# Efrat19/flink

Hardware: AMD Instinct MI355X
Metric: events/sec keyed sliding-window agg at 1/2/4/8 GPUs; % of HBM roofline (higher is better)
Workload: dtype int64

## Files before the change

flink_amd/csrc/gw_kernels.h:

```cpp
#pragma once
#include "gw_device.h"

namespace gw {

struct PaneTable {
    int64_t* base;
    int64_t cap;
    int64_t nreg;
    int64_t region_words;
    int32_t log2S;
    int32_t rb1;
    int32_t nsub;
    int32_t ring;
    int32_t words;
    int32_t agg;
    int32_t has_mask;
    int32_t mask_shift;
};

GW_HD int64_t pt_S(const PaneTable& t) { return (int64_t)1 << t.log2S; }
GW_HD int64_t* pt_region(const PaneTable& t, int64_t r) { return t.base + r * t.region_words; }
GW_HD int64_t* pt_key(const PaneTable& t, int64_t g) {
    return pt_region(t, g >> t.log2S) + (g & (pt_S(t) - 1));
}
// ... 113 lines not shown
    int32_t sr_bits;
    uint64_t apply_mask;
    uint64_t c_mask;
    const int64_t* c_rbeg;
    const uint32_t* c_r_row;
    const int64_t* c_r_base;
    int64_t* c_key;
    int32_t cur_empty;
    int64_t tile0;
    int64_t ntiles;
    int64_t ngroups;
    int32_t p2_group;
    int64_t* p1_key;
    int64_t* p1_a0;
    int64_t* p1_a1;
    uint8_t* p1_pos;
    uint32_t* p1_row;
    uint32_t* p2_desc;
    int64_t* p2_off;
    int64_t* p2_roff;
    int64_t* rbeg;
    int64_t* bk_off;
    int64_t* e_key;
    int64_t* e_a0;
    int64_t* e_a1;
    uint8_t* e_pos;
    uint32_t* r_row;
    int64_t* r_base;
    unsigned long long* batch_occ;
    DevStatus* st_host;
    unsigned long long st_seq;
    uint64_t ring_fresh;
    int32_t stale;
};

#ifndef GW_PART_TILE
#define GW_PART_TILE 4096
#endif
constexpr int kPartTile = GW_PART_TILE;
constexpr int kPartBuckets = 256;
constexpr int kRgnMaxRegions = 65536;
constexpr int kMaxGroup = 256;

struct MergeArgs {
    const int64_t* i_key;
    const int64_t* i_pane;
    const int64_t* i_a0;
    const int64_t* i_a1;
    int64_t n;
    int64_t b;
    int32_t b_pos;
    PaneTable t;
    int64_t* d_key;
    int64_t* d_pane;
    int64_t* d_a0;
    int64_t* d_a1;
    DevStatus* st;
};

constexpr uint32_t kOvTimer = 1;
constexpr uint32_t kOvDead = 2;
struct Overlay {
    const int32_t* head;
    const int64_t* key;
    const int64_t* k;
    const int64_t* a0;
// ... 63 lines not shown
    const int64_t* d_pane;
    const int64_t* d_a0;
    const int64_t* d_a1;
    int64_t n_def;
    int32_t max_p, kg_lo, kg_hi;
    int64_t* o_key;
    int64_t* o_pane;
    int64_t* o_a0;
    int64_t* o_a1;
    int32_t* o_kg;
    unsigned long long* n_out;
};
hipError_t launch_snap_collect(const SnapArgs& a, hipStream_t s);

hipError_t launch_table_init(const PaneTable& t, hipStream_t s);
hipError_t launch_overlay_attach(const PaneTable& t, const Overlay& ov, int32_t* head, DevStatus* st, hipStream_t s);
hipError_t launch_ingest(const IngestArgs& a, int path, int unroll, hipStream_t s);
hipError_t launch_region_p1(const IngestArgs& a, hipStream_t s, hipEvent_t e0 = nullptr, hipEvent_t e1 = nullptr);
hipError_t launch_publish_status(const IngestArgs& a, hipStream_t s);
hipError_t launch_region_flush(const IngestArgs& a, hipStream_t s, hipEvent_t e0 = nullptr, hipEvent_t e1 = nullptr);
hipError_t launch_region_collect(const IngestArgs& a, hipStream_t s);
int region_group(int d1_bits);
hipError_t launch_merge_deferred(const MergeArgs& a, hipStream_t s);
hipError_t launch_refire(const RefireArgs& a, hipStream_t s);
hipError_t launch_refire_keys(int mode, const int64_t* src, int64_t base, uint64_t* k, uint32_t* v, int64_t n,
                              hipStream_t s);
hipError_t launch_deferred_min(const int64_t* pane, int64_t n, DevStatus* st, hipStream_t s);
hipError_t launch_fire(const FireArgs& a, hipStream_t s, hipEvent_t e0 = nullptr, hipEvent_t e1 = nullptr);
struct FireGuard {
    unsigned long long expect_ndef;
    int64_t o_cap;
    int64_t nwin;
    int64_t reset_rows;
};
hipError_t launch_fire_guard(DevStatus* st, const FireGuard& g, hipStream_t s);
hipError_t launch_clean_stale(const PaneTable& t, uint64_t pmask, hipStream_t s);
hipError_t launch_evict(const EvictArgs& a, hipStream_t s);
hipError_t launch_rehash(const PaneTable& o, const PaneTable& n, DevStatus* st, hipStream_t s);
hipError_t launch_status_set(DevStatus* st, int word, unsigned long long v, int shard_field, hipStream_t s);
hipError_t launch_count_live(const PaneTable& t, unsigned long long* out, hipStream_t s);

hipError_t launch_key_groups(int64_t n, const int64_t* key, const int32_t* key_hash, int32_t max_p,
                             int32_t p, int32_t* kg, int32_t* owner, hipStream_t s);
int64_t partition_scratch_bytes(int64_t n, int32_t p);
hipError_t launch_check_keys(int64_t n, const int64_t* key, const int32_t* key_hash, int32_t max_p, int32_t kg_lo,
                             int32_t kg_hi, int check_range, unsigned long long* out, hipStream_t s);
constexpr int32_t kPartRegionMaxOwners = 16;
hipError_t launch_partition_regions(int64_t n, const int64_t* key, const int32_t* key_hash, const int64_t* ts,
                                    const int64_t* val, int32_t max_p, int32_t p, int64_t cap, int64_t* key_out,
                                    int64_t* ts_out, int64_t* val_out, int32_t* hash_out, const PackGeom* pack,
                                    uint64_t* packed_out, int64_t* counts, void* scratch, hipStream_t s,
                                    int turn = -1, int32_t nd_max = 0, int unstable = 0);
int64_t partition_regions_scratch_bytes(int64_t cap, int32_t nd);
hipError_t launch_partition(int64_t n, const int64_t* key, const int32_t* key_hash, const int64_t* ts,
                            const int64_t* val, int32_t max_p, int32_t p, int64_t* key_out,
                            int64_t* ts_out, int64_t* val_out, int64_t* counts, void* scratch,
                            hipStream_t s, int32_t* hash_out = nullptr, const PackGeom* pack = nullptr,
                            uint64_t* packed_out = nullptr);
hipError_t launch_select_lookup(int64_t n, const int64_t* sel, int64_t want, const int64_t* idx, const int64_t* dict,
                                int64_t dict_n, const int64_t* ts, int64_t* key_out, int64_t* ts_out, void* scratch,
                                hipStream_t s);
size_t select_lookup_scratch_bytes(int64_t n);
hipError_t launch_unpack(int64_t n, const uint64_t* w, const PackGeom& g, int64_t* key, int64_t* ts, int64_t* val,
                         hipStream_t s);

struct KeyHashMap {
    int64_t* key = nullptr;
    int32_t* hash = nullptr;
// ... 11 lines not shown
```

flink_amd/csrc/gw_pane.hip:

```cpp
#include <hip/hip_ext.h>
#include <type_traits>
#include "gw_kernels.h"

#include <algorithm>
#include <mutex>
#include <vector>

namespace gw {

template <int AGG>
__device__ __forceinline__ constexpr bool uses_mask() {
    return !(AGG == GW_COUNT || AGG == GW_AVG_I64 || AGG == GW_AVG_F64);
}

template <int AGG>
__device__ __forceinline__ uint64_t presence(const PaneTable& t, int64_t g) {
    if constexpr (uses_mask<AGG>()) {
        return pt_mask_get(t, g);
    } else {
        uint64_t m = 0;
        for (int r = 0; r < t.ring; ++r)
            if (pt_cell(t, g, r)[t.words - 1] != 0) m |= 1ull << r;
        return m;
    }
// ... 1304 lines not shown
        spills = marked;
    }
    __syncthreads();
    {
        const long2* sk = reinterpret_cast<const long2*>(lkeys);
        long2* dk = reinterpret_cast<long2*>(gkeys);
        for (int64_t w = threadIdx.x; w < S / 2; w += blockDim.x) {
            const int64_t line = w >> 3;
            if (s_kdirty[line >> 5] & (1u << (line & 31))) {
                const long2 v = sk[w];
                dk[w] = long2{slot_unhash((uint64_t)v.x), slot_unhash((uint64_t)v.y)};
            }
        }
    }
    if constexpr (M) copy_words((long long*)gmask, (const long long*)lmask, MW);
    for (int ai = 0; ai < 2; ++ai) {
        const int p = ai ? act1 : act0;
        if (p < 0) continue;
        copy_words((long long*)pt_cell(a.t, r << a.t.log2S, p), lcell + (int64_t)ai * S * W, S * W);
    }
    spills = wave_sum(spills);
    if (__lane_id() == 0 && spills) atomicAdd(&a.st->spills, spills);
    block_commit(a.st, 0, ins, flags, 0);
}

constexpr uint32_t kK32Empty = 0xffffffffu;
constexpr uint32_t kK32Foreign = 0xfffffffeu;
constexpr int kNarMaxF = 4;
constexpr int kNarMaxSlots = kNarMaxF * 2048;
constexpr int kNarLoadU = 4;
#ifndef GW_NAR_DEPTH
#define GW_NAR_DEPTH 2
#endif

__device__ __forceinline__ uint32_t k32_of(int64_t k) {
    return k == kEmptyKey ? kK32Empty : ((uint64_t)k < (uint64_t)kK32Foreign ? (uint32_t)k : kK32Foreign);
}

template <int AGG, bool STALE>
__global__ void __launch_bounds__(kApplyThreads) GW_APPLY_ATTR k_rgn_apply_nar(IngestArgs a) {
    if constexpr (!cmp_agg<AGG>()) {
        return;
    } else {
    extern __shared__ __attribute__((aligned(16))) unsigned char smem[];
    constexpr bool M = uses_mask<AGG>();
    constexpr bool N4 = AGG == GW_COUNT;
    constexpr int W = AGG == GW_AVG_I64 ? 2 : 1;
    __shared__ uint32_t r_cnt[kApplyRuns], r_src[kApplyRuns];
    __shared__ uint32_t s_kdirty[kNarMaxSlots / 16 / 32];
    __shared__ uint32_t s_pos;
    const int F = 1 << a.sr_bits;
    const int S = (int)pt_S(a.t), FS = F * S;
    const int l2S = a.t.log2S;
    const int64_t ncol = a.t.nsub >> a.sr_bits;
    const int64_t sr = blockIdx.x;
    const int64_t bucket = sr / ncol, col = sr - bucket * ncol;
    const int64_t rb0 = a.cur_empty ? 0 : a.rbeg[bucket], re0 = a.cur_empty ? 0 : a.rbeg[bucket + 1];
    const int64_t rb1 = a.c_mask ? a.c_rbeg[bucket] : 0, re1 = a.c_mask ? a.c_rbeg[bucket + 1] : 0;
    const int lane = threadIdx.x & 63, wave = threadIdx.x >> 6, nw = blockDim.x >> 6;
    uint32_t* lkeys = reinterpret_cast<uint32_t*>(smem);
    uint8_t* lmask = reinterpret_cast<uint8_t*>(lkeys + FS);
    long long* lcell = reinterpret_cast<long long*>(lmask + (M ? FS : 0));
    uint32_t* qk = reinterpret_cast<uint32_t*>(lcell + (int64_t)FS * W) + wave * kApplyQ;
    int32_t* qv = reinterpret_cast<int32_t*>(lcell + (int64_t)FS * W) + nw * kApplyQ + wave * kApplyQ;
    int qn = 0;
    const unsigned long long cur_pos = a.cur_empty ? 0ull : (*(volatile unsigned long long*)a.batch_occ) & a.apply_mask;
    struct List {
        const uint32_t* rows;
        const int64_t* rbase;
        const uint64_t* rk;
        const uint32_t* rk32;
        int64_t rb, re;
        unsigned long long pos;
    };
    const List list0{a.r_row, a.r_base, reinterpret_cast<const uint64_t*>(a.e_key),
                     reinterpret_cast<const uint32_t*>(a.e_key), rb0, re0, cur_pos & 0xffull};
    const List list1{a.c_r_row, a.c_r_base, reinterpret_cast<const uint64_t*>(a.c_key),
                     reinterpret_cast<const uint32_t*>(a.c_key), rb1, re1, a.c_mask & 0xffull};

    if (threadIdx.x == 0) s_pos = 0;
    for (int i = threadIdx.x; i < kNarMaxSlots / 16 / 32; i += blockDim.x) s_kdirty[i] = 0;
    __syncthreads();
    {
        uint32_t any = 0;
        for (int l = 0; l < 2; ++l) {
            const List L = l ? list1 : list0;
            for (int64_t rnd = L.rb + threadIdx.x; rnd < L.re; rnd += blockDim.x)
                for (unsigned long long pm = L.pos; pm; pm &= pm - 1) {
                    const int p = __ffsll((long long)pm) - 1;
                    if (L.rows[rnd * kPartBuckets + ((col << 3) | p)] & 0xffffu) any |= 1u << p;
                }
        }
        any = (uint32_t)wave_ior(any);
        if (lane == 0 && any) atomicOr(&s_pos, any);
    }
    __syncthreads();
    const uint32_t pmask = s_pos;
    if (!pmask) return;

    {
        const int nk2 = FS / 2, nm16 = M ? FS / 16 : 0, tot = nk2 + nm16;
        for (int w0 = threadIdx.x; w0 < tot; w0 += kNarLoadU * blockDim.x) {
            long2 v[kNarLoadU];
#pragma unroll
            for (int u = 0; u < kNarLoadU; ++u) {
                const int w = w0 + u * blockDim.x;
                v[u] = long2{0, 0};
                if (w < nk2) {
                    const int d = w >> (l2S - 1), j = w & (S / 2 - 1);
                    v[u] = reinterpret_cast<const long2*>(pt_region(a.t, sr * F + d))[j];
                } else if (w < tot) {
                    const int wm_ = w - nk2, d = wm_ >> (l2S - 4), j = wm_ & (S / 16 - 1);
                    v[u] = reinterpret_cast<const long2*>(pt_mask_base(a.t, sr * F + d))[j];
                }
            }
#pragma unroll
            for (int u = 0; u < kNarLoadU; ++u) {
                const int w = w0 + u * blockDim.x;
                if (w < nk2) {
                    reinterpret_cast<uint2*>(lkeys)[w] = uint2{k32_of(v[u].x), k32_of(v[u].y)};
                } else if (w < tot) {
                    reinterpret_cast<long2*>(lmask)[w - nk2] = v[u];
                }
            }
        }
    }
    unsigned long long ins = 0, flags = 0, spills = 0;

    auto probe_insert = [&](uint32_t k, uint64_t h) -> int {
        const int d = F > 1 ? (int)(pt_sub(a.t, h) & (F - 1)) : 0;
        uint32_t* kd = lkeys + d * S;
// ... 226 lines not shown
        for (int l = 0; l < 2; ++l) {
            const List L = l ? list1 : list0;
            for (unsigned long long pm = L.pos & pmask; pm; pm &= pm - 1) {
                const int p = __ffsll((long long)pm) - 1;
                const int64_t ccol = (col << 3) | p;
                for (int64_t rnd = L.rb + wave; rnd < L.re; rnd += nw) {
                    const uint32_t d = L.rows[rnd * kPartBuckets + ccol];
                    const int64_t src = L.rbase[rnd] + (d >> 16);
                    for (uint32_t k = lane; k < (d & 0xffffu); k += 64) {
                        const uint64_t r = N4 ? (uint64_t)L.rk32[src + k] : L.rk[src + k];
                        const uint32_t kk = N4 ? (uint32_t)(r >> 4) : (uint32_t)r;
                        const uint64_t h = slot_hash((int64_t)kk);
                        const int dd = F > 1 ? (int)(pt_sub(a.t, h) & (F - 1)) : 0;
                        int j = (int)(h & (uint64_t)(S - 1) & ~(uint64_t)(kProbeGroup - 1));
                        bool present = false;
                        for (int q = 0; q < S; ++q) {
                            const uint32_t x = lkeys[dd * S + j];
                            if (x == kk) { present = true; break; }
                            if (x == kK32Empty) break;
                            j = (j + 1) & (S - 1);
                        }
                        if (!present) {
                            if constexpr (N4) const_cast<uint32_t*>(L.rk32)[src + k] = (uint32_t)r | kNarSpill;
                            else const_cast<uint64_t*>(L.rk)[src + k] = r | ((uint64_t)kNarSpill << 32);
                            marked++;
                        }
                    }
                }
            }
        }
        spills = marked;
    }
    __syncthreads();
    if constexpr (M) {
        const int per = S / 16, lper = l2S - 4;
        for (int w = threadIdx.x; w < FS / 16; w += blockDim.x) {
            const int d = w >> lper;
            reinterpret_cast<long2*>(pt_mask_base(a.t, sr * F + d))[w - d * per] = reinterpret_cast<const long2*>(lmask)[w];
        }
    }
    for (int j = threadIdx.x; j < FS; j += blockDim.x) {
        const int line = j >> 4;
        if ((s_kdirty[line >> 5] >> (line & 31)) & 1u) {
            const uint32_t k = lkeys[j];
            if (k != kK32Foreign) {
                const int d = j >> l2S;
                pt_region(a.t, sr * F + d)[j - d * S] = k == kK32Empty ? kEmptyKey : (int64_t)k;
            }
        }
    }
    spills = wave_sum(spills);
    if (__lane_id() == 0 && spills) atomicAdd(&a.st->spills, spills);
    block_commit(a.st, 0, ins, flags, 0);
    }
}

template <int AGG>
__global__ void __launch_bounds__(256) k_rgn_collect_nar2(IngestArgs a) {
    constexpr bool N4 = AGG == GW_COUNT;
    const bool carry = blockIdx.y == 1;
    if (carry ? !a.c_mask : a.cur_empty) return;
    const int nb1 = 1 << a.d1_bits;
    const int64_t n = carry ? a.c_rbeg[kPartBuckets + 1 + nb1] : a.bk_off[nb1];
    int64_t* rk = carry ? a.c_key : a.e_key;
    uint32_t* rk32 = reinterpret_cast<uint32_t*>(rk);
    const int64_t stride = (int64_t)gridDim.x * blockDim.x;
    for (int64_t base = blockIdx.x * (int64_t)blockDim.x; base < n; base += stride) {
        const int64_t i = base + threadIdx.x;
        bool spill = false;
        int64_t key = 0, pane = 0, c0 = 0;
        if (i < n) {
            const uint64_t w = N4 ? (uint64_t)rk32[i] : (uint64_t)rk[i];
            const uint32_t lo = N4 ? (uint32_t)w : (uint32_t)(w >> 32);
            if (nar_spilled(lo)) {
                spill = true;
                if (N4) rk32[i] = (uint32_t)w & ~kNarSpill;
                else rk[i] = (int64_t)(w & ~((uint64_t)kNarSpill << 32));
                key = N4 ? nar_key32((uint32_t)w) : nar_key(w);
                c0 = N4 ? 1 : nar_val(w);
                const int64_t rel = ((int64_t)nar_pos(lo) - a.b_pos + a.t.ring) % a.t.ring;
                pane = a.p_late + (int64_t)a.delta + rel;
            }
        }
        defer_write(a, spill, key, pane, c0, 1);
    }
}
// ... 472 lines not shown
        load(A, c0);
        for (int64_t base = c0; base < c1; base += 2 * step) {
            const bool more = base + step < c1;
            if (more) load(B, base + step);
            fold(A, base);
            if (!more) break;
            if (base + 2 * step < c1) load(A, base + 2 * step);
            fold(B, base + step);
        }
    }
    flush();
}

template <int AGG>
__global__ void __launch_bounds__(256) k_clean_stale(PaneTable t, uint64_t pm) {
    if constexpr (uses_mask<AGG>()) {
        const int64_t id0 = identity0(AGG);
        for (int64_t g = blockIdx.x * (int64_t)blockDim.x + threadIdx.x; g < t.cap; g += (int64_t)gridDim.x * blockDim.x) {
            const uint64_t m = pt_mask_get(t, g);
            for (uint64_t q = pm & ~m; q; q &= q - 1) pt_cell(t, g, __ffsll((long long)q) - 1)[0] = id0;
        }
    }
}

__global__ void __launch_bounds__(64) k_fire_guard(DevStatus* st, FireGuard g) {
    const int lane = threadIdx.x;
    unsigned long long flags = 0, used = 0;
    for (int i = lane; i < kShards; i += 64) {
        flags |= st->sh[i].flags;
        used += st->sh[i].ins;
    }
    flags = wave_ior(flags);
    used = wave_sum(used);
    if (lane == 0) {
        if (g.reset_rows) st->rows = 0;
        const unsigned long long rows = g.reset_rows ? 0ull : st->rows;
        const bool skip = st->spills != 0 || st->wide_vals != 0 ||
                          (flags & (GW_DF_TABLE_FULL | GW_DF_NO_TS | GW_DF_RANGE)) != 0 ||
                          st->n_deferred != g.expect_ndef ||
                          (int64_t)rows + g.nwin * ((int64_t)used + 1) > g.o_cap;
        st->fire_skip = skip ? 1ull : 0ull;
        st->fire_rows0 = rows;
    }
}

template <int AGG>
__global__ void __launch_bounds__(256) k_evict(EvictArgs a) {
    const int64_t nslots = a.t.cap + 1;
    const int64_t stride = (int64_t)gridDim.x * blockDim.x;
    const int64_t id0 = identity0(AGG);
    const int W = a.t.words;
    if (blockIdx.x == 0 && threadIdx.x < kShards) atomicAnd(&a.st->sh[threadIdx.x].occ, ~a.emask);
    for (int64_t base = blockIdx.x * (int64_t)blockDim.x; base < nslots; base += stride) {
        const int64_t g = base + threadIdx.x;
        uint64_t m = 0;
        int64_t key = 0;
        if (g < nslots) {
            key = *pt_key(a.t, g);
            m = presence<AGG>(a.t, g) & a.emask;
        }
        unsigned long long off = wave_reserve_n(&a.st->n_deferred, (unsigned)__popcll(m));
        if (m) {
            if constexpr (uses_mask<AGG>()) pt_mask_put(a.t, g, pt_mask_get(a.t, g) & ~a.emask);
            while (m) {
                const int pos = __ffsll((long long)m) - 1;
                m &= m - 1;
                int64_t* c = pt_cell(a.t, g, pos);
                a.d_key[off] = key;
                a.d_pane[off] = a.pane_of_pos[pos];
                a.d_a0[off] = c[0];
                a.d_a1[off] = W == 2 ? c[1] : 0;
                off++;
                c[0] = id0;
                if (W == 2) c[1] = 0;
            }
// ... 231 lines not shown
        GW_TLAUNCH(k_rgn_plan1, dim3((unsigned)a.ngroups), dim3(256), 0, s, e0, nullptr, a);                   \
        hipLaunchKernelGGL(k_rgn_plan2, dim3((unsigned)nb1), dim3(256), 0, s, a);                              \
        hipLaunchKernelGGL(k_rgn_plan3, dim3(1), dim3(256), 0, s, a);                                          \
        hipLaunchKernelGGL((k_rgn_p2<A, CM>), dim3((unsigned)(a.ngroups * nb1)), dim3(kPartThreads), part_lds, s, \
                           a);                                                                                  \
    }                                                                                                           \
    GW_TLAUNCH((k_rgn_apply<A, CM>), dim3((unsigned)a.t.nreg), dim3(kApplyThreads), apply_lds, s,               \
               single ? e0 : nullptr, e1, a)
#define L(A)                        \
    if (a.fmt == kFmtNar) {         \
        L2(A, kFmtNar);             \
    } else if (a.fmt == kFmtCmp) {  \
        L2(A, kFmtCmp);             \
    } else {                        \
        L2(A, kFmtWide);            \
    }
    if (a.fmt == kFmtNar && a.nar2) {
        const int F = 1 << a.sr_bits;
        const int64_t FS = (int64_t)F * S;
        const bool M = a.t.has_mask != 0;
        const size_t lds = (size_t)FS * 4 + (M ? (size_t)FS : 0) + (size_t)FS * a.t.words * 8 +
                           (size_t)(kApplyThreads / 64) * kApplyQ * 8;
#define LN(A)                                                                                                   \
    lds_opt_in((const void*)k_rgn_p2<A, kFmtNar>, part_lds);                                                   \
    lds_opt_in((const void*)k_rgn_apply_nar<A, true>, lds);                                                   \
    lds_opt_in((const void*)k_rgn_apply_nar<A, false>, lds);                                                  \
    if (!a.cur_empty) {                                                                                         \
        GW_TLAUNCH(k_rgn_plan1, dim3((unsigned)a.ngroups), dim3(256), 0, s, e0, nullptr, a);                   \
        hipLaunchKernelGGL(k_rgn_plan2, dim3((unsigned)nb1), dim3(256), 0, s, a);                              \
        hipLaunchKernelGGL(k_rgn_plan3, dim3(1), dim3(256), 0, s, a);                                          \
        hipLaunchKernelGGL((k_rgn_p2<A, kFmtNar>), dim3((unsigned)(a.ngroups * nb1)), dim3(kPartThreads), part_lds, \
                           s, a);                                                                               \
    }                                                                                                           \
    if (a.stale)                                                                                                \
        GW_TLAUNCH((k_rgn_apply_nar<A, true>), dim3((unsigned)(a.t.nreg >> a.sr_bits)), dim3(kApplyThreads), lds, \
                   s, a.cur_empty ? e0 : nullptr, e1, a);                                                       \
    else                                                                                                        \
        GW_TLAUNCH((k_rgn_apply_nar<A, false>), dim3((unsigned)(a.t.nreg >> a.sr_bits)), dim3(kApplyThreads),     \
                   lds, s, a.cur_empty ? e0 : nullptr, e1, a)
        GW_AGG_SWITCH(a.t.agg, LN);
#undef LN
        return hipGetLastError();
    }
    GW_AGG_SWITCH(a.t.agg, L);
#undef L
#undef L2
    return hipGetLastError();
}

hipError_t launch_region_collect(const IngestArgs& a, hipStream_t s) {
    const int64_t n = a.ntiles * kPartTile;
#define L(A)                                                                                         \
    if (a.fmt == kFmtNar && a.nar2)                                                                  \
        hipLaunchKernelGGL(k_rgn_collect_nar2<A>, dim3(grid_for(n), 2), dim3(256), 0, s, a);        \
    else if (a.fmt == kFmtNar)                                                                       \
        hipLaunchKernelGGL(k_rgn_collect_nar<A>, dim3((unsigned)a.t.nreg), dim3(256), 0, s, a);     \
    else if (a.fmt == kFmtCmp)                                                                       \
        hipLaunchKernelGGL(k_rgn_collect_cmp<A>, dim3((unsigned)a.t.nreg), dim3(256), 0, s, a);     \
    else                                                                                             \
        hipLaunchKernelGGL(k_rgn_collect<A>, dim3(grid_for(n)), dim3(256), 0, s, a)
    GW_AGG_SWITCH(a.t.agg, L);
#undef L
    return hipGetLastError();
}

hipError_t launch_merge_deferred(const MergeArgs& a, hipStream_t s) {
#define L(A) hipLaunchKernelGGL(k_merge_deferred<A>, dim3(grid_for(a.n)), dim3(256), 0, s, a)
// ... 31 lines not shown
    if (a.ov.head == nullptr && npos >= 1 && npos <= 6 && a.nwin <= 255 &&
        (int64_t)a.nwin * kF2Threads * 2 <= kF2Stage) {
        const bool av = a.t.agg == GW_AVG_I64 || a.t.agg == GW_AVG_F64;
        const int64_t tile = (int64_t)kF2Threads * (av ? 1 : 2);
        const int fg = (int)std::min<int64_t>(1024, std::max<int64_t>(1, (a.t.cap + 1 + tile - 1) / tile));
#define F2(A, NPV) \
    GW_TLAUNCH((k_fire2<A, NPV, (A == GW_AVG_I64 || A == GW_AVG_F64) ? 1 : 2>), dim3(fg), dim3(kF2Threads), 0, s, e0, e1, a)
#define L(A)                      \
    switch (npos) {               \
    case 1: F2(A, 1); break;      \
    case 2: F2(A, 2); break;      \
    case 3: F2(A, 3); break;      \
    case 4: F2(A, 4); break;      \
    case 5: F2(A, 5); break;      \
    default: F2(A, 6); break;     \
    }
        GW_AGG_SWITCH(a.t.agg, L);
#undef L
#undef F2
        return hipGetLastError();
    }
    const int fg = (int)std::min<int64_t>(1024, std::max<int64_t>(1, (a.t.cap + 1 + 255) / 256));
#define L(A) GW_TLAUNCH(k_fire<A>, dim3(fg), dim3(256), 0, s, e0, e1, a)
    GW_AGG_SWITCH(a.t.agg, L);
#undef L
    return hipGetLastError();
}

hipError_t launch_fire_guard(DevStatus* st, const FireGuard& g, hipStream_t s) {
    hipLaunchKernelGGL(k_fire_guard, dim3(1), dim3(64), 0, s, st, g);
    return hipGetLastError();
}

hipError_t launch_clean_stale(const PaneTable& t, uint64_t pmask, hipStream_t s) {
    if (!t.has_mask || !pmask) return hipSuccess;
#define L(A) hipLaunchKernelGGL(k_clean_stale<A>, dim3(grid_for(t.cap)), dim3(256), 0, s, t, pmask)
    GW_AGG_SWITCH(t.agg, L);
#undef L
    return hipGetLastError();
}

hipError_t launch_evict(const EvictArgs& a, hipStream_t s) {
#define L(A) hipLaunchKernelGGL(k_evict<A>, dim3(grid_for(a.t.cap + 1)), dim3(256), 0, s, a)
    GW_AGG_SWITCH(a.t.agg, L);
#undef L
    return hipGetLastError();
}

hipError_t launch_status_set(DevStatus* st, int word, unsigned long long v, int shard_field, hipStream_t s) {
    hipLaunchKernelGGL(k_status_set, dim3(1), dim3(64), 0, s, st, word, v, shard_field);
    return hipGetLastError();
}

hipError_t launch_snap_collect(const SnapArgs& a, hipStream_t s) {
#define L(A) hipLaunchKernelGGL(k_snap_collect<A>, dim3(grid_for(a.t.cap + 1 + a.n_def)), dim3(256), 0, s, a)
    GW_AGG_SWITCH(a.t.agg, L);
#undef L
    return hipGetLastError();
}

hipError_t launch_overlay_attach(const PaneTable& t, const Overlay& ov, int32_t* head, DevStatus* st, hipStream_t s) {
    if (ov.n == 0) return hipSuccess;
    hipLaunchKernelGGL(k_overlay_attach, dim3(grid_for(ov.n)), dim3(256), 0, s, t, ov, head, st);
    return hipGetLastError();
}

// ... 12 lines not shown
```

flink_amd/csrc/gw_runtime.cpp:

```cpp
#include <hip/hip_runtime.h>

#include <algorithm>
#include <array>
#include <functional>
#include <map>
#include <set>
#include <atomic>
#include <chrono>
#include <thread>
#include <cstdarg>
#include <cstdio>
#include <cstdlib>
#include <cstring>
#include <new>
#include <string>
#include <tuple>
#include <vector>
#include <mutex>

#include "gw_first.h"
#include "gw_kernels.h"
#include "gw_netbuf.h"
#include "gw_session.h"
#include "gw_sort.h"
// ... 1176 lines not shown
    }

    bool compact_ok(int d1_bits) const {
        const int agg = cfg.agg;
        const bool int_agg = agg == GW_COUNT || agg == GW_SUM_I64 || agg == GW_SUM_I32 || agg == GW_MIN_I64 ||
                             agg == GW_MAX_I64 || agg == GW_AVG_I64;
        static const bool env_off = getenv("GW_NO_COMPACT") != nullptr;
        return int_agg && !cmp_off && !env_off && !gap_size && d1_bits >= 2 && (int64_t)tv.ring <= ((int64_t)1 << (d1_bits - 1));
    }
    int region_fmt(int d1_bits) const {
        const int agg = cfg.agg;
        const bool int_agg = agg == GW_COUNT || agg == GW_SUM_I64 || agg == GW_SUM_I32 || agg == GW_MIN_I64 ||
                             agg == GW_MAX_I64 || agg == GW_AVG_I64;
        static const bool nar_env_off = getenv("GW_NO_NARROW") != nullptr;
        static const bool cmp_env_off = getenv("GW_NO_COMPACT") != nullptr;
        if (int_agg && !gap_size && !cmp_env_off && !nar_off && !nar_env_off && !(cfg.flags & GW_FLAG_NO_NARROW) &&
            tv.ring <= 8)
            return 2;
        return compact_ok(d1_bits) ? 1 : 0;
    }

    struct PendingFlush {
        IngestArgs a;
        int64_t window_recs = 0;
    };
    int flush_buffer(uint64_t apply_mask = ~0ull) {
        PendingFlush pf;
        bool launched = false;
        int rc;
        if ((rc = flush_launch(apply_mask, pf, launched)) || !launched) return rc;
        if ((rc = refresh())) return rc;
        return flush_post(pf);
    }
    int flush_launch(uint64_t apply_mask, PendingFlush& pf, bool& launched) {
        launched = false;
        if (!nseg && !carry_on) return GW_OK;
        int rc;
        IngestArgs& a = pf.a;
        if ((rc = base_args(a, 0, nullptr, nullptr, nullptr))) return rc;
        region_args(a);
        if (carry_on && !a.nar2) return fail(GW_E_STATE, "internal: carried records without a nar2 flush");
        a.ntiles = buf_tiles;
        a.p2_group = region_group(a.d1_bits);
        a.ngroups = (buf_tiles + a.p2_group - 1) / a.p2_group;
        a.ring_fresh = buf_fresh;
        a.cur_empty = nseg == 0;
        if (carry_on) {
            const int c = eset ^ 1;
            a.c_mask = carry_mask;
            a.c_key = eset_key(c);
            a.c_r_row = eset_row(c);
            a.c_r_base = eset_base(c);
            a.c_rbeg = eset_rbeg(c);
        }
        uint64_t carry_next = 0;
        static const bool carry_off = [] { const char* e = getenv("GW_NAR_CARRY"); return e && atoi(e) == 0; }();
        if (a.nar2 && nseg && apply_mask != ~0ull && cfg.allowed_lateness == 0 && ov_n == 0 && !carry_off) {
            const uint64_t ring = R >= 64 ? ~0ull : ((1ull << R) - 1);
            carry_next = ring & ~apply_mask;
            a.apply_mask = apply_mask;
            if (carry_next && (rc = ensure_eset2())) return rc;
        }
        const int64_t window_recs = buf_recs;
        nseg = 0;
        buf_tiles = 0;
        buf_recs = 0;
        carry_on = false;
        if (carry_next) {
            carry_on = true;
            carry_mask = carry_next;
            eset ^= 1;
        }
        if (timing) {
            auto ev = t_apply.get();
            HIPCHECK(launch_region_flush(a, stream, ev.first, ev.second));
            t_apply.pending.push_back(ev);
        } else {
            HIPCHECK(launch_region_flush(a, stream));
        }
        HIPCHECK(hipMemsetAsync(d_tmp + 1, 0, 8, stream));
        occ_zeroed = true;
        stats.applies++;
        dirty = true;
        launched = true;
        pf.window_recs = window_recs;
        return GW_OK;
    }
    int flush_post(PendingFlush& pf) {
        int rc;
        IngestArgs& a = pf.a;
        if (h_st->wide_vals) {
            if (h_st->wide_vals * 64 > (unsigned long long)pf.window_recs) {
                if (a.fmt == 2) nar_off = true;
                else cmp_off = true;
            }
            if ((rc = set_field(offsetof(DevStatus, wide_vals), 0))) return rc;
        }
        if (h_st->spills) {
            if ((rc = ensure_deferred((int64_t)h_st->n_deferred + (int64_t)h_st->spills))) return rc;
            if ((rc = set_field(offsetof(DevStatus, spills), 0))) return rc;
            HIPCHECK(launch_region_collect(a, stream));
            dirty = true;
            if ((rc = refresh())) return rc;
            if (!(h_st->flags & GW_DF_TABLE_FULL) && (rc = merge_deferred())) return rc;
// ... 1079 lines not shown
            hd.gap != cfg.gap || hd.size != cfg.size || hd.slide != cfg.slide ||
            hd.max_parallelism != cfg.max_parallelism || hd.reserved != (int32_t)ew)
            return fail(GW_E_INVALID, "snapshot of a different window / aggregate / max parallelism");
        const int64_t nk = (int64_t)hd.kg_hi - hd.kg_lo + 1;
        const int64_t hdr = (int64_t)sizeof hd + (nk + 1) * 8;
        if (nk <= 0 || hd.entries < 0 || len < hdr || hd.entries > (len - hdr) / (ew * 8))
            return fail(GW_E_INVALID, "truncated snapshot blob");
        const int64_t* in = (const int64_t*)((const char*)buf + hdr);
        std::vector<int64_t> ent, hkeys;
        std::vector<int32_t> hvals;
        ent.reserve((size_t)(hd.entries * ew0));
        for (int64_t i = 0; i < hd.entries; ++i) {
            const size_t at = ent.size();
            ent.resize(at + (size_t)ew0);
            memcpy(ent.data() + at, (const char*)in + i * ew * 8, (size_t)ew0 * 8);
            if (hashed) {
                int64_t hw;
                memcpy(&hw, (const char*)in + (i * ew + ew0) * 8, 8);
                hkeys.push_back(ent[at]);
                hvals.push_back((int32_t)hw);
            }
        }
        int rc = khm_check_host(hkeys, hvals);
        if (rc || dry) return rc;
        rc = session_restore(sess, ent.data(), hd.entries, err);
        if (rc) return fail(rc, "%s", err.c_str());
        return khm_insert_host(hkeys, hvals);
    }

#ifndef GW_FAST_FIRE
#define GW_FAST_FIRE 1
#endif
    int64_t fast_fires = 0;
    int fast_fire(i128 kt, uint64_t need, bool& done) {
        done = false;
        int rc;
        const bool eligible = GW_FAST_FIRE && ov_n == 0 && !rf_bound && occ != 0 && h_st->n_deferred == 0;
        const i128 k_first = fired_k;
        if (eligible) {
            const i128 kl = floor_div(ring_min() - n, m) + 1;
            if (kl > k_first || k_first * m < B || floor_div(k_first * m + R - n, m) < kt) return flush_buffer(need);
        } else {
            return flush_buffer(need);
        }
        PendingFlush pf;
        bool launched = false;
        if ((rc = flush_launch(need, pf, launched))) return rc;
        const i128 B0 = B;
        const uint64_t stale0 = stale_pos;
        B = k_first * m;
        FireArgs f{};
        i128 keep;
        if ((rc = fire_args(k_first, kt, (kt + 1) * m, f, keep))) return rc;
        f.o_key = o_key; f.o_start = o_start; f.o_end = o_end; f.o_res = o_res;
        f.guarded = 1;
        lazy_retire(f);
        FireGuard g{0, o_cap, (int64_t)f.nwin, rows_reset_pending ? 1 : 0};
        rows_reset_pending = false;
        HIPCHECK(launch_fire_guard(d_st, g, stream));
        if ((rc = fire_launch(f))) return rc;
        dirty = true;
        if ((rc = refresh())) return rc;
        if (!h_st->fire_skip) {
            fired(f, kt, keep);
            dirty = false;
            occ = h_st->occ;
            fast_fires++;
            done = true;
            return GW_OK;
        }
        B = B0;
        stale_pos = stale0;
        if (timing) t_fire.drop_last();
        return launched ? flush_post(pf) : GW_OK;
    }

    int advance_pane(int64_t w, int64_t* rows_out) {
        int rc;
        if (rows_out) *rows_out = 0;
        if (w <= wm) return GW_OK;
        if ((rc = ov_finalize())) return rc;
        const i128 kt = k_for_wm(w);
        const i128 ct = clean_k_at(w);
        int64_t before = 0;
        if (cfg.allowed_lateness > 0) {
            if ((rc = ensure_fresh())) return rc;
            before = (int64_t)h_st->rows;
            if (rf_bound && (rc = process_refire())) return rc;
            if (kt < fired_k && !(occ && ct * m > B)) {
// ... 2148 lines not shown
    return GW_OK;
}

void* gw_stream(gw_handle* h) { return h ? (void*)h->stream : nullptr; }

int gw_enable_kernel_timing(gw_handle* h, int enable) {
    if (!h) return GW_E_INVALID;
    for (gw_handle* kid : h->kids) gw_enable_kernel_timing(kid, enable);
    h->timing = enable != 0;
    h->timing_every = enable > 1 ? enable : 1;
    h->timing_ctr = 0;
    if (h->sess) session_enable_timing(h->sess, h->timing);
    return GW_OK;
}

int gw_kernel_time_ms(gw_handle* h, int which, double* ms, int64_t* launches) {
    if (!h) return GW_E_INVALID;
    if (!h->kids.empty()) {
        double total = 0;
        int64_t l0 = 0;
        for (size_t j = 0; j < h->kids.size(); ++j) {
            double m = 0;
            int64_t l = 0;
            gw_kernel_time_ms(h->kids[j], which, &m, &l);
            total += m * (double)l;
            if (j == 0) l0 = l;
        }
        if (ms) *ms = l0 ? total / (double)l0 : 0.0;
        if (launches) *launches = l0;
        return GW_OK;
    }
    hipStreamSynchronize(h->stream);
    if (h->sess) return session_kernel_time(h->sess, which, ms, launches);
    if (which == 3) {
        if (ms) *ms = 0.0;
        if (launches) *launches = h->fast_fires;
        return GW_OK;
    }
    KernelTimer& t = which == 0 ? h->t_ingest : which == 1 ? h->t_fire : h->t_apply;
    t.resolve();
    if (ms) *ms = t.launches ? t.total_ms / (double)t.launches : 0.0;
    if (launches) *launches = t.launches;
    t.total_ms = 0;
    t.launches = 0;
    return GW_OK;
}

int gw_window_stagger_offset(int32_t stagger, int64_t processing_time, double random01, int64_t size,
                             int64_t global_offset, int64_t* offset_out) {
    if (!offset_out || size <= 0 || global_offset <= -size || global_offset >= size) return GW_E_INVALID;
    int64_t st = 0;
    switch (stagger) {
    case GW_STAGGER_ALIGNED: break;
    case GW_STAGGER_RANDOM:
        if (!(random01 >= 0.0 && random01 < 1.0)) return GW_E_INVALID;
        st = (int64_t)(random01 * (double)size);
        break;
    case GW_STAGGER_NATURAL: {
        const int64_t rem = processing_time % size;
        const int64_t start = processing_time - (rem < 0 ? rem + size : rem);
        st = std::max<int64_t>(0, processing_time - start);
        break;
    }
    default: return GW_E_INVALID;
    }
    *offset_out = (global_offset + st) % size;
    return GW_OK;
}

// ... 148 lines not shown
```

Baseline: 55.60 billion.

## Fuse window fire into region apply kernel for single-window fast fires

Adds a FIRE variant of the NAR region apply kernel. While the freshly applied pane cells are still in LDS, it folds the window's panes and emits output rows directly, and a separate retire kernel clears the fired positions afterwards. This avoids a second full pass over the pane table in the standalone fire kernel. In exchange it adds guard logic that can revoke the fused result and fall back to the normal path, and it only applies to sum and count aggregations with at most 6 panes per window.

```diff
diff --git a/flink_amd/csrc/gw_kernels.h b/flink_amd/csrc/gw_kernels.h
--- a/flink_amd/csrc/gw_kernels.h
+++ b/flink_amd/csrc/gw_kernels.h
@@ -169,6 +169,15 @@
     unsigned long long st_seq;
     uint64_t ring_fresh;
     int32_t stale;
+    int32_t fire;
+    uint64_t f_wmask;
+    int64_t f_start;
+    int64_t f_end;
+    int64_t* o_key;
+    int64_t* o_start;
+    int64_t* o_end;
+    int64_t* o_res;
+    int64_t o_cap;
 };
 
 #ifndef GW_PART_TILE
@@ -298,8 +307,10 @@
     int64_t o_cap;
     int64_t nwin;
     int64_t reset_rows;
+    int64_t after;
 };
 hipError_t launch_fire_guard(DevStatus* st, const FireGuard& g, hipStream_t s);
+hipError_t launch_fire_retire(const FireArgs& a, hipStream_t s);
 hipError_t launch_clean_stale(const PaneTable& t, uint64_t pmask, hipStream_t s);
 hipError_t launch_evict(const EvictArgs& a, hipStream_t s);
 hipError_t launch_rehash(const PaneTable& o, const PaneTable& n, DevStatus* st, hipStream_t s);
diff --git a/flink_amd/csrc/gw_pane.hip b/flink_amd/csrc/gw_pane.hip
--- a/flink_amd/csrc/gw_pane.hip
+++ b/flink_amd/csrc/gw_pane.hip
@@ -1360,14 +1360,22 @@
 #ifndef GW_NAR_DEPTH
 #define GW_NAR_DEPTH 2
 #endif
+#ifndef GW_FIRE_U
+#define GW_FIRE_U 2
+#endif
 
 __device__ __forceinline__ uint32_t k32_of(int64_t k) {
     return k == kEmptyKey ? kK32Empty : ((uint64_t)k < (uint64_t)kK32Foreign ? (uint32_t)k : kK32Foreign);
 }
 
-template <int AGG, bool STALE>
+template <int AGG>
+__device__ __forceinline__ constexpr bool fire_agg() {
+    return AGG == GW_SUM_I64 || AGG == GW_SUM_I32 || AGG == GW_COUNT;
+}
+
+template <int AGG, bool STALE, bool FIRE = false>
 __global__ void __launch_bounds__(kApplyThreads) GW_APPLY_ATTR k_rgn_apply_nar(IngestArgs a) {
-    if constexpr (!cmp_agg<AGG>()) {
+    if constexpr (!cmp_agg<AGG>() || (FIRE && !fire_agg<AGG>())) {
         return;
     } else {
     extern __shared__ __attribute__((aligned(16))) unsigned char smem[];
@@ -1424,7 +1432,7 @@
     }
     __syncthreads();
     const uint32_t pmask = s_pos;
-    if (!pmask) return;
+    if (!pmask && !FIRE) return;
 
     {
         const int nk2 = FS / 2, nm16 = M ? FS / 16 : 0, tot = nk2 + nm16;
@@ -1717,7 +1725,7 @@
         spills = marked;
     }
     __syncthreads();
-    if constexpr (M) {
+    if (M && pmask) {
         const int per = S / 16, lper = l2S - 4;
         for (int w = threadIdx.x; w < FS / 16; w += blockDim.x) {
             const int d = w >> lper;
@@ -1737,6 +1745,132 @@
     spills = wave_sum(spills);
     if (__lane_id() == 0 && spills) atomicAdd(&a.st->spills, spills);
     block_commit(a.st, 0, ins, flags, 0);
+    if constexpr (FIRE) {
+        static_assert(W == 1 && kNarMaxSlots / 64 <= kApplyRuns && kNarMaxSlots / 64 <= 128, "fused fire geometry");
+        uint32_t* s_fc = r_cnt;
+        __shared__ unsigned long long s_fbase;
+        if (threadIdx.x == 0) s_fbase = *(volatile unsigned long long*)&a.st->fire_skip;
+        __threadfence_block();
+        __syncthreads();
+        if (s_fbase) return;
+        const uint64_t wm = a.f_wmask;
+        const int npos = __popcll(wm);
+        const int lp = pmask ? 31 - __clz((int)pmask) : -1;
+        int posl[6];
+        {
+            uint64_t need = wm;
+#pragma unroll
+            for (int q = 0; q < 6; ++q) {
+                posl[q] = need ? __ffsll((long long)need) - 1 : 0;
+                need &= need - 1;
+            }
+        }
+        const int nchunk = FS >> 6;
+        constexpr int FU = GW_FIRE_U;
+        for (int c0 = wave; c0 < nchunk; c0 += FU * nw) {
+            int64_t v[FU][6];
+#pragma unroll
+            for (int u = 0; u < FU; ++u) {
+                const int c = c0 + u * nw;
+                const int slot = min(c, nchunk - 1) << 6 | lane;
+                const int64_t g = ((sr * F + (slot >> l2S)) << l2S) | (slot & (S - 1));
+#pragma unroll
+                for (int q = 0; q < 6; ++q) {
+                    v[u][q] = id0;
+                    if (q < npos && posl[q] != lp) v[u][q] = __builtin_nontemporal_load(pt_cell(a.t, g, posl[q]));
+                }
+            }
+#pragma unroll
+            for (int u = 0; u < FU; ++u) {
+                const int c = c0 + u * nw;
+                if (c >= nchunk) break;
+                const int slot = c << 6 | lane;
+                const uint32_t mb = M ? lmask[slot] : 0u;
+                const int64_t vl = lcell[slot];
+                int64_t r0 = id0, r1 = 0;
+                bool any = false;
+#pragma unroll
+                for (int q = 0; q < 6; ++q) {
+                    if (q >= npos) break;
+                    const int64_t x = posl[q] == lp ? vl : v[u][q];
+                    const bool pres = M ? ((mb >> posl[q]) & 1) != 0 : x != 0;
+                    if (pres) {
+                        fold_cell(AGG, r0, r1, x, 0);
+                        any = true;
+                    }
+                }
+                lcell[slot] = any ? cell_result(AGG, r0, r1) : 0;
+                const uint64_t bal = __ballot(any);
+                if (lane == 0) s_fc[c] = (uint32_t)__popcll(bal);
+            }
+        }
+        __syncthreads();
+        if (wave == 0) {
+            const uint32_t n0 = 2 * lane < nchunk ? s_fc[2 * lane] : 0u;
+            const uint32_t n1 = 2 * lane + 1 < nchunk ? s_fc[2 * lane + 1] : 0u;
+            uint32_t incl = n0 + n1;
+            for (int o = 1; o < 64; o <<= 1) {
+                const uint32_t up = __shfl_up(incl, o);
+                if (lane >= o) incl += up;
+            }
+            s_fc[2 * lane] = incl - n0 - n1;
+            s_fc[2 * lane + 1] = incl - n1;
+            if (lane == 63) {
+                unsigned long long base = 0;
+                if (incl) {
+                    base = atomicAdd(&a.st->rows, (unsigned long long)incl);
+                    if (base + incl > (unsigned long long)a.o_cap) {
+                        atomicExch(&a.st->fire_skip, 1ull);
+                        base = ~0ull;
+                    }
+                }
+                s_fbase = base;
+            }
+        }
+        if (blockIdx.x == 0 && threadIdx.x == 0) {
+            const int64_t g = a.t.cap;
+            const uint64_t mb = M ? pt_mask_get(a.t, g) : ~0ull;
+            int64_t r0 = id0, r1 = 0;
+            bool any = false;
+            for (uint64_t q = wm; q; q &= q - 1) {
+                const int pos = __ffsll((long long)q) - 1;
+                const int64_t x = *pt_cell(a.t, g, pos);
+                if (M ? ((mb >> pos) & 1) != 0 : x != 0) {
+                    fold_cell(AGG, r0, r1, x, 0);
+                    any = true;
+                }
+            }
+            if (any) {
+                const unsigned long long j = atomicAdd(&a.st->rows, 1ull);
+                if (j < (unsigned long long)a.o_cap) {
+                    a.o_key[j] = kEmptyKey;
+                    a.o_start[j] = a.f_start;
+                    a.o_end[j] = a.f_end;
+                    a.o_res[j] = cell_result(AGG, r0, r1);
+                } else {
+                    atomicExch(&a.st->fire_skip, 1ull);
+                }
+            }
+        }
+        __syncthreads();
+        const unsigned long long base = s_fbase;
+        if (base == ~0ull) return;
+        for (int c = wave; c < nchunk; c += nw) {
+            const int slot = c << 6 | lane;
+            const int64_t res = lcell[slot];
+            const bool any = M ? (lmask[slot] & wm) != 0 : res != 0;
+            const uint64_t bal = __ballot(any);
+            if (any) {
+                const unsigned long long j = base + s_fc[c] + (unsigned)__popcll(bal & ((1ull << lane) - 1ull));
+                const uint32_t k = lkeys[slot];
+                const int64_t k64 = k == kK32Foreign ? pt_region(a.t, sr * F + (slot >> l2S))[slot & (S - 1)] : (int64_t)k;
+                __builtin_nontemporal_store(k64, &a.o_key[j]);
+                __builtin_nontemporal_store(a.f_start, &a.o_start[j]);
+                __builtin_nontemporal_store(a.f_end, &a.o_end[j]);
+                __builtin_nontemporal_store(res, &a.o_res[j]);
+            }
+        }
+    }
     }
 }
 
@@ -2275,7 +2409,13 @@
     }
     flags = wave_ior(flags);
     used = wave_sum(used);
-    if (lane == 0) {
+    if (lane == 0 && g.after) {
+        const bool skip = st->fire_skip != 0 || st->spills != 0 || st->wide_vals != 0 ||
+                          (flags & (GW_DF_TABLE_FULL | GW_DF_NO_TS | GW_DF_RANGE)) != 0 ||
+                          st->n_deferred != g.expect_ndef;
+        if (skip) st->rows = st->fire_rows0;
+        st->fire_skip = skip ? 1ull : 0ull;
+    } else if (lane == 0) {
         if (g.reset_rows) st->rows = 0;
         const unsigned long long rows = g.reset_rows ? 0ull : st->rows;
         const bool skip = st->spills != 0 || st->wide_vals != 0 ||
@@ -2284,6 +2424,47 @@
                           (int64_t)rows + g.nwin * ((int64_t)used + 1) > g.o_cap;
         st->fire_skip = skip ? 1ull : 0ull;
         st->fire_rows0 = rows;
+    }
+}
+
+template <int AGG>
+__global__ void __launch_bounds__(256) k_fire_retire(FireArgs a) {
+    if (*(volatile unsigned long long*)&a.st->fire_skip) return;
+    constexpr bool M = uses_mask<AGG>();
+    constexpr int W = (AGG == GW_AVG_I64 || AGG == GW_AVG_F64) ? 2 : 1;
+    if (blockIdx.x == 0 && threadIdx.x < kShards) atomicAnd(&a.st->sh[threadIdx.x].occ, ~a.rmask);
+    if (!a.rmask) return;
+    const int64_t id0 = identity0(AGG);
+    const int64_t stride = (int64_t)gridDim.x * blockDim.x, t0 = blockIdx.x * (int64_t)blockDim.x + threadIdx.x;
+    if (t0 == 0) {
+        const int64_t g = a.t.cap;
+        if constexpr (M) pt_mask_put(a.t, g, pt_mask_get(a.t, g) & ~a.rmask);
+        for (uint64_t m = a.rmask; m; m &= m - 1) {
+            int64_t* c = pt_cell(a.t, g, __ffsll((long long)m) - 1);
+            c[0] = id0;
+            if (W == 2) c[1] = 0;
+        }
+    }
+    if constexpr (M) {
+        uint64_t rep = a.rmask;
+        for (int b = 8 << a.t.mask_shift; b < 64; b <<= 1) rep |= rep << b;
+        const int64_t MW = pt_mask_words(a.t);
+        for (int64_t i = t0; i < a.t.nreg * MW; i += stride) {
+            const int64_t r = i / MW;
+            uint64_t* p = reinterpret_cast<uint64_t*>(pt_mask_base(a.t, r)) + (i - r * MW);
+            const uint64_t v = *p;
+            if (v & rep) *p = v & ~rep;
+        }
+    }
+    if (!(M && a.lazy_retire)) {
+        for (uint64_t m = a.rmask; m; m &= m - 1) {
+            const int pos = __ffsll((long long)m) - 1;
+            for (int64_t g = t0; g < a.t.cap; g += stride) {
+                int64_t* c = pt_cell(a.t, g, pos);
+                c[0] = id0;
+                if (W == 2) c[1] = 0;
+            }
+        }
     }
 }
 
@@ -2581,7 +2762,11 @@
         hipLaunchKernelGGL((k_rgn_p2<A, kFmtNar>), dim3((unsigned)(a.ngroups * nb1)), dim3(kPartThreads), part_lds, \
                            s, a);                                                                               \
     }                                                                                                           \
-    if (a.stale)                                                                                                \
+    if (a.fire) {                                                                                               \
+        lds_opt_in((const void*)k_rgn_apply_nar<A, true, true>, lds);                                          \
+        GW_TLAUNCH((k_rgn_apply_nar<A, true, true>), dim3((unsigned)(a.t.nreg >> a.sr_bits)),                  \
+                   dim3(kApplyThreads), lds, s, a.cur_empty ? e0 : nullptr, e1, a);                             \
+    } else if (a.stale)                                                                                         \
         GW_TLAUNCH((k_rgn_apply_nar<A, true>), dim3((unsigned)(a.t.nreg >> a.sr_bits)), dim3(kApplyThreads), lds, \
                    s, a.cur_empty ? e0 : nullptr, e1, a);                                                       \
     else                                                                                                        \
@@ -2679,6 +2864,14 @@
     return hipGetLastError();
 }
 
+hipError_t launch_fire_retire(const FireArgs& a, hipStream_t s) {
+    const int64_t n = a.t.has_mask && a.lazy_retire ? a.t.nreg * pt_mask_words(a.t) : a.t.cap;
+#define L(A) hipLaunchKernelGGL(k_fire_retire<A>, dim3(grid_for(n)), dim3(256), 0, s, a)
+    GW_AGG_SWITCH(a.t.agg, L);
+#undef L
+    return hipGetLastError();
+}
+
 hipError_t launch_clean_stale(const PaneTable& t, uint64_t pmask, hipStream_t s) {
     if (!t.has_mask || !pmask) return hipSuccess;
 #define L(A) hipLaunchKernelGGL(k_clean_stale<A>, dim3(grid_for(t.cap)), dim3(256), 0, s, t, pmask)
diff --git a/flink_amd/csrc/gw_runtime.cpp b/flink_amd/csrc/gw_runtime.cpp
--- a/flink_amd/csrc/gw_runtime.cpp
+++ b/flink_amd/csrc/gw_runtime.cpp
@@ -1232,7 +1232,7 @@
         if ((rc = refresh())) return rc;
         return flush_post(pf);
     }
-    int flush_launch(uint64_t apply_mask, PendingFlush& pf, bool& launched) {
+    int flush_launch(uint64_t apply_mask, PendingFlush& pf, bool& launched, const FireArgs** fuse = nullptr) {
         launched = false;
         if (!nseg && !carry_on) return GW_OK;
         int rc;
@@ -1270,6 +1270,19 @@
             carry_on = true;
             carry_mask = carry_next;
             eset ^= 1;
+        }
+        if (fuse && *fuse && !(a.nar2 && a.fmt == 2)) *fuse = nullptr;
+        if (fuse && *fuse) {
+            const FireArgs& f = **fuse;
+            a.fire = 1;
+            a.f_wmask = f.wmask[0];
+            a.f_start = f.start0;
+            a.f_end = f.start0 + f.size;
+            a.o_key = o_key; a.o_start = o_start; a.o_end = o_end; a.o_res = o_res;
+            a.o_cap = o_cap;
+            FireGuard g{0, o_cap, 1, rows_reset_pending ? 1 : 0};
+            rows_reset_pending = false;
+            HIPCHECK(launch_fire_guard(d_st, g, stream));
         }
         if (timing) {
             auto ev = t_apply.get();
@@ -2415,6 +2428,8 @@
 #define GW_FAST_FIRE 1
 #endif
     int64_t fast_fires = 0;
+    int64_t fused_fires = 0;
+    int64_t fused_revoked = 0;
     int fast_fire(i128 kt, uint64_t need, bool& done) {
         done = false;
         int rc;
@@ -2428,7 +2443,20 @@
         }
         PendingFlush pf;
         bool launched = false;
-        if ((rc = flush_launch(need, pf, launched))) return rc;
+        static const bool fused_off = [] { const char* e = getenv("GW_FUSED_FIRE"); return e && atoi(e) == 0; }();
+        const FireArgs* fuse = nullptr;
+        FireArgs ff{};
+        if (!fused_off && kt == k_first && (nseg || carry_on) && n <= 6 &&
+            (cfg.agg == GW_COUNT || (tv.has_mask && (cfg.agg == GW_SUM_I64 || cfg.agg == GW_SUM_I32)))) {
+            const i128 Bs = B;
+            i128 keep_;
+            B = k_first * m;
+            rc = fire_args(k_first, kt, (kt + 1) * m, ff, keep_);
+            B = Bs;
+            if (rc) return rc;
+            fuse = &ff;
+        }
+        if ((rc = flush_launch(need, pf, launched, &fuse))) return rc;
         const i128 B0 = B;
         const uint64_t stale0 = stale_pos;
         B = k_first * m;
@@ -2438,6 +2466,26 @@
         f.o_key = o_key; f.o_start = o_start; f.o_end = o_end; f.o_res = o_res;
         f.guarded = 1;
         lazy_retire(f);
+        if (fuse && launched) {
+            FireGuard g2{0, o_cap, 1, 0, 1};
+            HIPCHECK(launch_fire_guard(d_st, g2, stream));
+            HIPCHECK(launch_fire_retire(f, stream));
+            dirty = true;
+            if ((rc = refresh())) return rc;
+            if (!h_st->fire_skip) {
+                fired(f, kt, keep);
+                dirty = false;
+                occ = h_st->occ;
+                fast_fires++;
+                fused_fires++;
+                done = true;
+                return GW_OK;
+            }
+            fused_revoked++;
+            B = B0;
+            stale_pos = stale0;
+            return flush_post(pf);
+        }
         FireGuard g{0, o_cap, (int64_t)f.nwin, rows_reset_pending ? 1 : 0};
         rows_reset_pending = false;
         HIPCHECK(launch_fire_guard(d_st, g, stream));
@@ -4652,9 +4700,9 @@
     }
     hipStreamSynchronize(h->stream);
     if (h->sess) return session_kernel_time(h->sess, which, ms, launches);
-    if (which == 3) {
+    if (which >= 3 && which <= 5) {
         if (ms) *ms = 0.0;
-        if (launches) *launches = h->fast_fires;
+        if (launches) *launches = which == 3 ? h->fast_fires : which == 4 ? h->fused_fires : h->fused_revoked;
         return GW_OK;
     }
     KernelTimer& t = which == 0 ? h->t_ingest : which == 1 ? h->t_fire : h->t_apply;
```

Measured after the change: 58.01 billion (median of 6 runs). 4.3% higher.
